# monkey0head/RePlay_cql

Measured on AMD Instinct MI355X. Metric: CQL train-steps/sec, higher is better.
Workload: dtype bf16; 1 GPU; BASELINE.json configs[2]: synthetic 1000000 users x 100000 items, CQL d=128, L=50, B=4096/GPU, bf16 MFMA + fp32 accumulate; users=1000000, items=100000, d=128, window=50, batch_per_gpu=4096, global_batch=4096, parallelism=dp1 (users sharded by rank, RCCL gradient all-reduce), k=10, dp_variant=single

## Files before the change

### include/cqlrec.h

```cpp
#ifndef CQLREC_H
#define CQLREC_H
#include <stdint.h>
#ifdef __cplusplus
extern "C" {
#endif

#define CQLREC_OK 0
#define CQLREC_ERR_INVALID (-1)
#define CQLREC_ERR_HIP (-2)
#define CQLREC_ABI_VERSION 2
#define CQLREC_SEG_ALIGN 64

typedef void* cqlrec_stream;

int cqlrec_abi_version(void);
const char* cqlrec_last_error(void);

typedef struct cqlrec_layout {
  int64_t n_items;
  int32_t d;
  int32_t reserved;
  int64_t off_E_in, off_E_out, off_b_out, off_W1, off_b1, off_W2, off_b2;
  int64_t total;
} cqlrec_layout;
// ... 65 lines not shown
                           cqlrec_stream stream);

int cqlrec_adam_ema(float* theta, float* grads, float* m, float* v, float* target, uint16_t* theta_b,
                    uint16_t* target_b, int64_t n, float step_size, float sqrt_bc2, float beta1, float beta2,
                    float eps, float tau, int32_t zero_grads, cqlrec_stream stream);
int cqlrec_cast_bf16(const float* src, uint16_t* dst_b, int64_t n, cqlrec_stream stream);

int64_t cqlrec_topk_ws_bytes(int64_t n_users, int64_t n_cand, int32_t d, int32_t k);
int cqlrec_score_topk(const uint16_t* H_b, int64_t n_users, const uint16_t* E_b, const float* b, int64_t n_cand,
                      int32_t d, const int32_t* item_ids, const int64_t* seen_off, const int32_t* seen_items,
                      const int32_t* seen_rows, int32_t k, void* ws, int64_t ws_bytes, int32_t* out_idx,
                      float* out_val, int32_t* out_cnt, cqlrec_stream stream);
#define CQLREC_TOPK_ALL 0
#define CQLREC_TOPK_SEEN 1
#define CQLREC_TOPK_SCORE 2
#define CQLREC_TOPK_SEEN_BESIDE 3
int cqlrec_score_topk_phase(const uint16_t* H_b, int64_t n_users, const uint16_t* E_b, const float* b, int64_t n_cand,
                            int32_t d, const int32_t* item_ids, const int64_t* seen_off, const int32_t* seen_items,
                            const int32_t* seen_rows, int32_t k, void* ws, int64_t ws_bytes, int32_t* out_idx,
                            float* out_val, int32_t* out_cnt, int32_t phase, cqlrec_stream stream);

int cqlrec_topk_seen_form(const void* ws, int64_t n_users, int64_t n_cand, int32_t d, int32_t k,
                          int32_t* out , cqlrec_stream stream);

#define CQLREC_SIM_DOT 0
#define CQLREC_SIM_COSINE 1
#define CQLREC_SIM_EUCLID 2
#define CQLREC_ITEM_KNN_MAX_K 512
int cqlrec_item_norms(const uint16_t* E_b, int64_t n_rows, int32_t d, float* norms, cqlrec_stream stream);
int64_t cqlrec_item_knn_ws_bytes(int64_t n_query, int64_t n_cand, int32_t d, int32_t k);
int cqlrec_item_knn(const uint16_t* E_b, const float* norms, int64_t n_rows, int32_t d, const int32_t* query_rows,
                    int64_t n_query, const int32_t* cand_rows, int64_t n_cand, int32_t metric, int32_t k, void* ws,
                    int64_t ws_bytes, int32_t* out_idx, float* out_val, int32_t* out_cnt, cqlrec_stream stream);

#define CQLREC_PAIRS_MAX_K 512
int64_t cqlrec_pairs_topk_ws_bytes(int64_t n_sel, int64_t nnz, int32_t d, int32_t k);
int cqlrec_pairs_topk(const uint16_t* H_b, const uint16_t* E_b, const float* b, int64_t n_items, int32_t d,
                      const int64_t* pair_off, const int32_t* pair_items, const int32_t* rows, int64_t n_sel,
                      const int64_t* seen_off, const int32_t* seen_items, int32_t k, void* ws, int64_t ws_bytes,
                      float* out_score, int32_t* out_idx, float* out_val, int32_t* out_cnt, cqlrec_stream stream);

typedef struct cqlrec_train_ctx {
  cqlrec_layout layout;
  const int64_t* offsets;
  const int32_t* items;
  const float* rewards;
// ... 350 lines not shown
```

### replay_cql_amd/build.py

```python
from __future__ import annotations

import os
import shutil
import subprocess
import sys
from concurrent.futures import ThreadPoolExecutor
from pathlib import Path

PKG = Path(__file__).resolve().parent
CSRC = PKG / "csrc"
LIB = PKG / "libcqlrec.so"
TORCH_LIB = PKG / "libcqlrec_torch.so"
SOURCES = ["library.hip", "state_side.hip", "adam.hip", "qhead.hip", "qhead_de.hip", "qhead_de2.hip", "qhead_de3.hip", "qhead_argmax2.hip", "qhead_fwd2.hip", "qhead_fwd3.hip", "qhead_topk2.hip", "qhead_topk4.hip", "select_common.hip", "segment_common.hip", "topk.hip", "item_knn.hip", "pairs_topk.hip", "gbwd.hip", "prep.hip", "metrics.hip", "split.hip", "prepare.hip", "features.hip", "neighbour.hip", "als.hip", "dense.hip", "slim.hip", "step_streams.hip", "train.hip"]
EXTRA = {
    "state_side.hip": ["-ffp-contract=off"],
    "adam.hip": ["-ffp-contract=off"],
    "qhead.hip": ["-mllvm", "-amdgpu-mfma-vgpr-form=1"],
    "qhead_de.hip": ["-mllvm", "-amdgpu-mfma-vgpr-form=1"],
    "qhead_de2.hip": ["-mllvm", "-amdgpu-mfma-vgpr-form=1"],
    "qhead_de3.hip": ["-mllvm", "-amdgpu-mfma-vgpr-form=1"],
    "qhead_argmax2.hip": ["-mllvm", "-amdgpu-mfma-vgpr-form=1"],
    "qhead_topk2.hip": ["-mllvm", "-amdgpu-mfma-vgpr-form=1"],
    "qhead_topk4.hip": ["-mllvm", "-amdgpu-mfma-vgpr-form=1"],
    "qhead_fwd2.hip": ["-mllvm", "-amdgpu-mfma-vgpr-form=1"],
    "qhead_fwd3.hip": ["-mllvm", "-amdgpu-mfma-vgpr-form=1"],
    "topk.hip": ["-mllvm", "-amdgpu-mfma-vgpr-form=1"],
    "item_knn.hip": ["-ffp-contract=off", "-mllvm", "-amdgpu-mfma-vgpr-form=1"],
    "pairs_topk.hip": ["-ffp-contract=off"],
    "split.hip": ["-ffp-contract=off"],
    "prepare.hip": ["-ffp-contract=off"],
    "features.hip": ["-ffp-contract=off"],
    "neighbour.hip": ["-ffp-contract=off"],
    "als.hip": ["-ffp-contract=off"],
    "dense.hip": ["-ffp-contract=off", "-mllvm", "-amdgpu-mfma-vgpr-form=1"],
    "slim.hip": ["-ffp-contract=off"],
}
ARCH = "gfx950"


def _hipcc() -> str:
    for cand in (os.environ.get("HIPCC"), shutil.which("hipcc"), "/opt/rocm/bin/hipcc"):
        if cand and Path(cand).exists():
            return cand
    raise RuntimeError("hipcc not found (set HIPCC or install ROCm)")


# ... 99 lines not shown
```

### replay_cql_amd/csrc/qhead_internal.h

```cpp
#pragma once
#include "common.h"
#include "qde_pieces.h"

#define QM_LSE 1
#define QM_ARGMAX 2
#define QM_TILEMAX 3
#define QM_BWD_DH 4
#define QM_LSE_DH 6
#define QM_TOPK 7
#define QM_TOPK10 8
#define QS_TOPK_K 16
#define QS_TOPK_BUF 4

#define QS_TI 64
#define QS_SPW_FWD 2
#define QS_SPW_BWD 1
#define QS_TARGET_BLOCKS 768
#define QS_TARGET_BLOCKS_BWD 512
#define QS_REF_MARGIN 5.5f
#ifndef QS_NBUF
#define QS_NBUF 3
#endif
#ifndef QS_NBUF_BWD
#define QS_NBUF_BWD 2
// ... 47 lines not shown
                   int accumulate, hipStream_t s, CqlAdamFix* defer = nullptr, const float* nlse_nat = nullptr);

int cql_qde_fixup_deferred(const CqlAdamFix& f, float* out, float* out_cs, hipStream_t s);
int cql_qhead_bwd_items_long(const uint16_t* H_b, const float* nlse2, const float* coef, const int32_t* act, int64_t batch,
                             const uint16_t* E_out_b, const float* b_out, int64_t n_items, int32_t d, float scale, void* ws,
                             int64_t ws_bytes, float* g_E_out, float* g_b_out, hipStream_t stream, CqlAdamFix* defer,
                             const float* nlse_nat);

struct QTk2Args {
  const uint16_t* H_b;
  int64_t n_users;
  const uint16_t* E_b;
  const float* bias;
  int64_t n_cand;
  int64_t split_rows;
  int nsplit;
  const uint32_t* seen_bits;
  unsigned long long* keys;
  int k;
  const uint32_t* seen_lists;
  const uint16_t* seen_lists_ovf;
  const uint32_t* guard;
  int guard_want;
};
bool cql_topk2_supported(int d, int k, int64_t n_cand);
void cql_topk2_split(int64_t n_users, int64_t n_cand, int* nsplit, int64_t* split_rows);
int64_t cql_topk2_bits_bytes(int64_t n_users, int64_t n_cand);
const uint32_t* cql_topk2_lists_word(const uint32_t* bits, int64_t n_users, int64_t n_cand);
int cql_topk2_seen_bits(const int64_t* seen_off, const int32_t* seen_items, const int32_t* seen_rows, int64_t n_users,
                        int64_t n_cand, uint32_t* bits, hipStream_t s, int beside_scoring = 0);
int cql_topk2_run(const QTk2Args& a, int d, hipStream_t s);
bool cql_topk4_use(int d, int k, int64_t n_users, int64_t n_cand);
int cql_topk4_run(const QTk2Args& a, hipStream_t s);
bool cql_topk4_lists_on();
bool cql_topk4_lists_fit(int64_t n_users, int64_t n_cand, int64_t space_bytes);
int cql_topk4_seen_lists(const int64_t* seen_off, const int32_t* seen_items, const int32_t* seen_rows, int64_t n_users,
                         int64_t n_cand, void* space, int64_t space_bytes, uint32_t* flag, hipStream_t s);

int cql_qhead_argmax_step(const uint16_t* H_b, int64_t rows, const uint16_t* E_out_b, const float* b_out, int64_t n_items,
                          int32_t d, void* ws, int64_t ws_bytes, float* out_val, int32_t* out_idx, hipStream_t stream);

struct QFwd2Args {
  const uint16_t* H_b;
  int64_t n_states;
  const uint16_t* E_b;
  const float* bias;
  int64_t n_items;
// ... 16 lines not shown
```

### replay_cql_amd/csrc/qhead_topk2.hip

```cpp
#include <stdlib.h>
#include <type_traits>
#include "qhead_image.h"

#define TK2_Q 24
#define TK2_K 16
#define TK2_NBUF 3
static_assert(TK2_K == QS_TOPK_K, "list format shared with topk_merge_kernel");

typedef __attribute__((address_space(3))) unsigned long long lds_u64;
typedef __attribute__((ext_vector_type(2))) unsigned int u32x2;
typedef __attribute__((address_space(3))) u32x2 lds_u2;

template <int D>
struct Tk2Cfg {
  using C = DeCfg<D, 4>;
  static constexpr int STRIPS = 4 * 256;
  static constexpr int SEEN = 4 * 512;
  static constexpr int BUF = C::STAGE_BYTES + STRIPS + SEEN;
  static constexpr int RING = TK2_NBUF * BUF;
  static constexpr int QUEUES = 4 * 2 * TK2_Q * 512;
  static constexpr int SMEM = RING + QUEUES;
  static constexpr int VPS = C::LPS + 2;
};

// ... 32 lines not shown
template <int D, int KC>
__global__ __launch_bounds__(256, 1) void qtopk2_kernel(QTk2Args a) {
  static_assert(KC == 10 || KC == 16, "lists of 10 or 16 sorted keys");
  using T = Tk2Cfg<D>;
  using C = typename T::C;
  constexpr int KS = C::KS;
  static_assert(C::TILES == 2 && T::VPS == 6, "two tiles per stage, six pieces per wave (tk2_wait_stages)");
  extern __shared__ __attribute__((aligned(16))) unsigned char smem[];

  const int tid = threadIdx.x, lane = tid & 63;
  const int wave = __builtin_amdgcn_readfirstlane(tid >> 6);
  const int r = lane & 31, h = lane >> 5;
  const int split = blockIdx.x % a.nsplit;
  const int64_t rblk = blockIdx.x / a.nsplit;
  const int64_t res0 = rblk * 256 + wave * 64;
  const int64_t s_begin = (int64_t)split * a.split_rows;
  const int64_t s_end = (s_begin + a.split_rows < a.n_cand) ? (s_begin + a.split_rows) : a.n_cand;
  const int nstage = (s_end > s_begin) ? (int)((s_end - s_begin + C::TI - 1) / C::TI) : 0;
  const uint32_t gstage0 = (uint32_t)(s_begin / C::TI);

  bf16x8 rf[2][KS];
#pragma unroll
  for (int g = 0; g < 2; ++g) load_owner_frags<D>(a.H_b, res0 + g * 32 + r, a.n_users, h, rf[g]);
  owner_fence();

  __amdgpu_buffer_rsrc_t rs_e = make_rsrc(a.E_b, a.n_cand * C::ROWB), rs_b = make_rsrc(a.bias, a.n_cand * 4);
  const int64_t nst_all = (a.n_cand + C::TI - 1) / C::TI;
  const bool has_seen = a.seen_bits != nullptr && res0 < a.n_users;
  const uint32_t* wsrc = has_seen ? a.seen_bits + (res0 >> 6) * nst_all * 128 : (const uint32_t*)a.bias;
  __amdgpu_buffer_rsrc_t rs_w =
      make_rsrc(wsrc, has_seen ? nst_all * 512 : 0);
  const uint32_t voff = img_stage_voff<C>(lane, wave, 0);
  const uint32_t voff4 = (uint32_t)lane * 4;
  const uint32_t smem_base = lds_addr_of(smem);
  auto issue_piece = [&](int stage, int buf, int pc) __attribute__((always_inline)) {
    const uint32_t bufp = __builtin_amdgcn_readfirstlane(smem_base + buf * T::BUF);
    const uint32_t gs = gstage0 + (uint32_t)stage;
    if (pc < C::LPS) bdma16(voff, rs_e, gs * C::STAGE_BYTES + C::PSTEP * pc, bufp + (4 * pc + wave) * 1024);
    else if (pc == C::LPS) bdma4(voff4, rs_b, gs * (C::TI * 4), bufp + C::STAGE_BYTES + wave * 256);
    else bdma16_lo32(4 * voff4, rs_w, gs * 512, bufp + C::STAGE_BYTES + T::STRIPS + wave * 512);
  };
  auto issue = [&](int stage, int buf) __attribute__((always_inline)) {
#pragma unroll
    for (int pc = 0; pc < T::VPS; ++pc) issue_piece(stage, buf, pc);
  };

// ... 1 lines not shown
  const ImgRead o = img_read_offsets<C>(lane);
  const int oa0 = o.oa0, oa1 = o.oa1;
  const int os = C::STAGE_BYTES + wave * 256 + 16 * h;
  const int ow = C::STAGE_BYTES + T::STRIPS + wave * 512 + r * 8;
  const lds_u8 *pA0, *pA1, *pS, *pW;
  const lds_u8 *nA0, *nA1, *nS;
  int boff_c = 0, boff_n = T::BUF;
  auto set_ptrs = [&]() __attribute__((always_inline)) {
    pA0 = lbase + boff_c + oa0; pA1 = lbase + boff_c + oa1; pS = lbase + boff_c + os; pW = lbase + boff_c + ow;
    nA0 = lbase + boff_n + oa0; nA1 = lbase + boff_n + oa1; nS = lbase + boff_n + os;
  };
  set_ptrs();

  lds_u8* qb[2];
  uint32_t la[2][2 * TK2_K];
  float thr[2];
  int cnt[2];
#pragma unroll
  for (int g = 0; g < 2; ++g) {
    qb[g] = (lds_u8*)smem + T::RING + ((wave * 2 + g) * TK2_Q * 64 + lane) * 8;
#ifdef TK2_ABL_NOSLOW
    thr[g] = 3.0e38f;
#else
    thr[g] = -3.0e38f;
#endif
    cnt[g] = 0;
#pragma unroll
    for (int j = 0; j < 2 * TK2_K; ++j) TK2_AW(la[g][j], 0u);
  }
  const int kth = a.k - 1;
  const bool kb0 = kth & 1, kb1 = kth & 2, kb2 = kth & 4, kb3 = kth & 8;

  auto merge = [&](auto G_) __attribute__((always_inline)) {
    constexpr int g = decltype(G_)::value;
    unsigned long long lst[TK2_K];
#pragma unroll
    for (int j = 0; j < TK2_K; ++j) {
      if (j < KC) {
        uint32_t lo, hi;
        TK2_AR(lo, la[g][2 * j]);
        TK2_AR(hi, la[g][2 * j + 1]);
        lst[j] = ((unsigned long long)hi << 32) | lo;
      } else {
        lst[j] = 0ull;
      }
    }
#pragma unroll 1
// ... 6 lines not shown
        kx = gt ? lst[j] : kx;
        lst[j] = hi_;
      }
    }
#pragma unroll
    for (int j = 0; j < KC; ++j) {
      TK2_AW(la[g][2 * j], (uint32_t)lst[j]);
      TK2_AW(la[g][2 * j + 1], (uint32_t)(lst[j] >> 32));
    }
    cnt[g] = 0;
    const unsigned long long m0 = kb0 ? ~0ull : 0ull, m1 = kb1 ? ~0ull : 0ull, m2 = kb2 ? ~0ull : 0ull,
                             m3 = kb3 ? ~0ull : 0ull;
    unsigned long long t8[8], t4[4], t2[2];
#pragma unroll
    for (int j = 0; j < 8; ++j) t8[j] = (lst[2 * j + 1] & m0) | (lst[2 * j] & ~m0);
#pragma unroll
    for (int j = 0; j < 4; ++j) t4[j] = (t8[2 * j + 1] & m1) | (t8[2 * j] & ~m1);
#pragma unroll
    for (int j = 0; j < 2; ++j) t2[j] = (t4[2 * j + 1] & m2) | (t4[2 * j] & ~m2);
    const unsigned long long kk = (t2[1] & m3) | (t2[0] & ~m3);
    const uint32_t okey = (uint32_t)(kk >> 32);
    const float own = (kk != 0ull) ? f32_from_order_key(okey) : -3.0e38f;
    const float own_up = (kk != 0ull) ? f32_from_order_key(okey + 1u) : -3.0e38f;
    thr[g] = fmaxf(own_up, __shfl_xor(own, 32));
  };

  auto slow = [&](const f32x16& acc, auto G_, int64_t trow0, uint32_t w) __attribute__((always_inline)) {
    constexpr int g = decltype(G_)::value;
    if (__builtin_amdgcn_ballot_w64(cnt[g] > TK2_Q - 16) != 0) merge(G_);
    float qm[4];
#pragma unroll
    for (int q = 0; q < 4; ++q) qm[q] = tk2_max4(acc[4 * q], acc[4 * q + 1], acc[4 * q + 2], acc[4 * q + 3]);
    const uint32_t wh = w >> (4 * h);
    const int lim = (int)((s_end - trow0 < 64) ? (s_end - trow0) : 64) - 4 * h;
    const uint32_t nrow = ~((uint32_t)trow0 + 4u * (uint32_t)h);
#pragma unroll
    for (int q = 0; q < 4; ++q) {
      if (__builtin_amdgcn_ballot_w64(qm[q] >= thr[g]) == 0) continue;
#pragma unroll
      for (int jj = 0; jj < 4; ++jj) {
        const int i = 4 * q + jj;
        const int rc = 8 * q + jj;
        const bool c0 = acc[i] >= thr[g];
        if (__builtin_amdgcn_ballot_w64(c0) == 0) continue;
        if (c0) {
          uint32_t whv = wh, nrv = nrow;
          int limv = lim;
// ... 298 lines not shown
```

### replay_cql_amd/csrc/qhead_topk4.hip

```cpp
#include <stdlib.h>
#include <type_traits>
#include "qhead_image.h"

#define TK4_G 4
#define TK4_Q 12
#define TK4_K 16
#define TK4_NBUF 3
#define TK4_SLOT_WORDS 64
#define TK4_SLOT_CAP 124
static_assert(TK4_K == QS_TOPK_K, "list format shared with topk_merge_kernel");

typedef __attribute__((address_space(3))) unsigned long long lds_u64_4;
typedef __attribute__((ext_vector_type(2))) unsigned int u32x2_4;
typedef __attribute__((address_space(3))) u32x2_4 lds_u2_4;
typedef __attribute__((address_space(3))) unsigned int lds_u32_4;
typedef __attribute__((address_space(3))) u32x4 lds_u4_4;

template <int D>
struct Tk4Cfg {
  using C = DeCfg<D, 4>;
  static constexpr int STRIP = 256;
  static constexpr int SEEN = 4 * 1024;
  static constexpr int BUF = C::STAGE_BYTES + STRIP + SEEN;
  static constexpr int RING = TK4_NBUF * BUF;
// ... 33 lines not shown
  using C = typename T::C;
  constexpr int KS = C::KS;
  static_assert(D == 128 && C::TILES == 2 && C::LPS == 4, "d = 128: two tiles per stage, four row pieces per wave");
  extern __shared__ __attribute__((aligned(16))) unsigned char smem[];

  const int tid = threadIdx.x, lane = tid & 63;
  const int wave = __builtin_amdgcn_readfirstlane(tid >> 6);
  const int r = lane & 31, h = lane >> 5;
  const int split = blockIdx.x % a.nsplit;
  const int64_t rblk = blockIdx.x / a.nsplit;
  const int64_t res0 = rblk * 512 + wave * 128;
  const int64_t s_begin = (int64_t)split * a.split_rows;
  const int64_t s_end = (s_begin + a.split_rows < a.n_cand) ? (s_begin + a.split_rows) : a.n_cand;
  const int nstage = (s_end > s_begin) ? (int)((s_end - s_begin + C::TI - 1) / C::TI) : 0;
  const uint32_t gstage0 = (uint32_t)(s_begin / C::TI);

  u32x4 rfa[TK4_G][KS];
#pragma unroll
  for (int g = 0; g < TK4_G; ++g) {
    int64_t row = res0 + g * 32 + r;
    if (row >= a.n_users) row = a.n_users - 1;
#pragma unroll
    for (int s = 0; s < KS; ++s) rfa[g][s] = *reinterpret_cast<const u32x4*>(a.H_b + row * D + 16 * s + 8 * h);
  }
  owner_fence();

  __amdgpu_buffer_rsrc_t rs_e = make_rsrc(a.E_b, a.n_cand * C::ROWB), rs_b = make_rsrc(a.bias, a.n_cand * 4);
  const int64_t nst_all = (a.n_cand + C::TI - 1) / C::TI;
  const int64_t nblk64 = LISTS ? (a.n_users + 127) / 128 : (a.n_users + 63) / 64;
  const int64_t blk0 = LISTS ? (res0 >> 7) : (res0 >> 6);
  const uint32_t* const seen_src = LISTS ? a.seen_lists : a.seen_bits;
  const bool has_seen = seen_src != nullptr && blk0 < nblk64;
  const uint32_t* wsrc = has_seen ? seen_src + blk0 * nst_all * (LISTS ? 64 : 128) : (const uint32_t*)a.bias;
  const bool two_blocks = !LISTS && has_seen && (blk0 + 1 < nblk64);
  const int64_t w_records = has_seen ? (LISTS ? nst_all * 256 : (two_blocks ? 2 : 1) * nst_all * 512) : 0;
  const uint64_t wp = (uint64_t)wsrc;
  const uint64_t wp_u = ((uint64_t)(uint32_t)__builtin_amdgcn_readfirstlane((int)(uint32_t)(wp >> 32)) << 32) |
                        (uint32_t)__builtin_amdgcn_readfirstlane((int)(uint32_t)wp);
  __amdgpu_buffer_rsrc_t rs_w = __builtin_amdgcn_make_buffer_rsrc((void*)wp_u, 0, __builtin_amdgcn_readfirstlane((int)w_records),
                                                                  0x00020000);
  const uint32_t voff_w = LISTS ? (uint32_t)lane * 4u
                                : (uint32_t)((lane >> 5) * (uint32_t)(nst_all * 512) + (lane & 31) * 16);
  const uint32_t voff = img_stage_voff<C>(lane, wave, 0);
  const uint32_t voff4 = (uint32_t)lane * 4;
  const uint32_t smem_base = lds_addr_of(smem);
  auto issue_piece = [&](int stage, int buf, int pc) __attribute__((always_inline)) {
// ... 11 lines not shown
  const lds_u8* lbase = (const lds_u8*)smem;
  const ImgRead o = img_read_offsets<C>(lane);
  const int oa0 = o.oa0, oa1 = o.oa1;
  const int os = C::STAGE_BYTES + 16 * h;
  const int ow = C::STAGE_BYTES + T::STRIP + wave * 1024 + r * 8;
  const lds_u8 *pA0, *pA1, *pS, *pW;
  const lds_u8 *nA0, *nA1, *nS;
  int boff_c = 0, boff_n = T::BUF;
  auto set_ptrs = [&]() __attribute__((always_inline)) {
    pA0 = lbase + boff_c + oa0; pA1 = lbase + boff_c + oa1; pS = lbase + boff_c + os; pW = lbase + boff_c + ow;
    nA0 = lbase + boff_n + oa0; nA1 = lbase + boff_n + oa1; nS = lbase + boff_n + os;
  };
  set_ptrs();

  uint32_t la[TK4_G][2 * TK4_K];
  float thr[TK4_G];
  int cnt[TK4_G];
  lds_u8* const qb0 = (lds_u8*)smem + T::RING + ((wave * TK4_G) * TK4_Q * 64 + lane) * 8;
#pragma unroll
  for (int g = 0; g < TK4_G; ++g) {
#ifdef TK4_ABL_NOSLOW
    thr[g] = 3.0e38f;
#else
    thr[g] = -3.0e38f;
#endif
    cnt[g] = 0;
#pragma unroll
    for (int j = 0; j < 2 * TK4_K; ++j) TK4_AW(la[g][j], 0u);
  }
  const int kth = a.k - 1;
  const bool kb0 = kth & 1, kb1 = kth & 2, kb2 = kth & 4, kb3 = kth & 8;

  auto merge = [&](auto G_) __attribute__((always_inline)) {
    constexpr int g = decltype(G_)::value;
    lds_u8* const qb = qb0 + g * (TK4_Q * 512);
    unsigned long long lst[TK4_K];
#pragma unroll
    for (int j = 0; j < TK4_K; ++j) {
      if (j < KC) {
        uint32_t lo, hi;
        TK4_AR(lo, la[g][2 * j]);
        TK4_AR(hi, la[g][2 * j + 1]);
        lst[j] = ((unsigned long long)hi << 32) | lo;
      } else {
        lst[j] = 0ull;
      }
    }
// ... 12 lines not shown
    for (int j = 0; j < KC; ++j) {
      TK4_AW(la[g][2 * j], (uint32_t)lst[j]);
      TK4_AW(la[g][2 * j + 1], (uint32_t)(lst[j] >> 32));
    }
    cnt[g] = 0;
    unsigned long long kk;
    if (kth == KC - 1) {
      kk = lst[KC - 1];
    } else {
      const unsigned long long m0 = kb0 ? ~0ull : 0ull, m1 = kb1 ? ~0ull : 0ull, m2 = kb2 ? ~0ull : 0ull,
                               m3 = kb3 ? ~0ull : 0ull;
      unsigned long long t8[8], t4[4], t2[2];
#pragma unroll
      for (int j = 0; j < 8; ++j) t8[j] = (lst[2 * j + 1] & m0) | (lst[2 * j] & ~m0);
#pragma unroll
      for (int j = 0; j < 4; ++j) t4[j] = (t8[2 * j + 1] & m1) | (t8[2 * j] & ~m1);
#pragma unroll
      for (int j = 0; j < 2; ++j) t2[j] = (t4[2 * j + 1] & m2) | (t4[2 * j] & ~m2);
      kk = (t2[1] & m3) | (t2[0] & ~m3);
    }
    const uint32_t okey = (uint32_t)(kk >> 32);
    const float own = (kk != 0ull) ? f32_from_order_key(okey) : -3.0e38f;
    const float own_up = (kk != 0ull) ? f32_from_order_key(okey + 1u) : -3.0e38f;
    thr[g] = fmaxf(own_up, __shfl_xor(own, 32));
  };

  auto slow = [&](const f32x16& acc, auto G_, int64_t trow0, uint32_t w) __attribute__((always_inline)) {
    constexpr int g = decltype(G_)::value;
    lds_u8* const qb = qb0 + g * (TK4_Q * 512);
    const uint32_t wh = w >> (4 * h);
    const int lim = (int)((s_end - trow0 < 64) ? (s_end - trow0) : 64) - 4 * h;
    const uint32_t nrow = ~((uint32_t)trow0 + 4u * (uint32_t)h);
    uint32_t qmask = 0u;
    {
      const float m0 = tk4_max4(acc[0], acc[1], acc[2], acc[3]), m1 = tk4_max4(acc[4], acc[5], acc[6], acc[7]);
      const float m2 = tk4_max4(acc[8], acc[9], acc[10], acc[11]), m3 = tk4_max4(acc[12], acc[13], acc[14], acc[15]);
      qmask = (__builtin_amdgcn_ballot_w64(m0 >= thr[g]) != 0 ? 1u : 0u) | (__builtin_amdgcn_ballot_w64(m1 >= thr[g]) != 0 ? 2u : 0u) |
              (__builtin_amdgcn_ballot_w64(m2 >= thr[g]) != 0 ? 4u : 0u) | (__builtin_amdgcn_ballot_w64(m3 >= thr[g]) != 0 ? 8u : 0u);
    }
#pragma unroll 1
    while (qmask != 0u) {
      const int q = __builtin_ctz(qmask);
      qmask &= qmask - 1u;
      float e[4];
#ifdef TK4_ABL_QUAD_SELECT
      const bool q1 = q & 1, q2 = q & 2;
#pragma unroll
// ... 410 lines not shown
```

### replay_cql_amd/csrc/topk.hip

```cpp
#include <stdlib.h>
#include "qhead_internal.h"
#include "select_common.h"

#define TK_CB_SMALL 1024
#define TK_CB_LARGE 4096
#define TK_MAX_K 2048
#define TK_SEEN_LDS 512

template <int D, int KPL, int TK_CB>
__global__ __launch_bounds__(64) void topk_select_kernel(const uint16_t* __restrict__ H_b, int64_t n_users,
                                                         const uint16_t* __restrict__ E_b, const float* __restrict__ b,
                                                         int64_t n_cand, const int32_t* __restrict__ item_ids,
                                                         const int64_t* __restrict__ seen_off,
                                                         const int32_t* __restrict__ seen_items,
                                                         const int32_t* __restrict__ seen_rows,
                                                         const float* __restrict__ tm_t, int gstride, int ngroups,
                                                         int tg, int k, int32_t* __restrict__ out_idx,
                                                         float* __restrict__ out_val, int32_t* __restrict__ out_cnt) {
  constexpr int KS = D / 16;
  __shared__ uint32_t hist[256];
  __shared__ float scores[32];
  __shared__ uint64_t cand[TK_CB];
  __shared__ int32_t seen_lds[TK_SEEN_LDS];

// ... 449 lines not shown
                            int32_t* out_idx, float* out_val, int32_t* out_cnt, hipStream_t s) {
  if (2 * nsplit <= 4)
    hipLaunchKernelGGL(topk_merge_wave_kernel, dim3(cql_ceil_div(n_users, 4)), dim3(256), 0, s, keys, nsplit, n_users,
                       item_ids, k, out_idx, out_val, out_cnt);
  else
    hipLaunchKernelGGL(topk_merge_kernel, dim3(cql_ceil_div(n_users, 256)), dim3(256), 0, s, keys, nsplit, n_users, item_ids,
                       k, out_idx, out_val, out_cnt);
}

static inline int64_t tk_bits_words(int64_t n_cand) { return ((n_cand + 31) / 32 + 3) / 4 * 4; }
#define TK_FUSED_MAX_SPLIT 32
static QSplit tk_fused_split(int64_t n_cand, int64_t n_users, int d) {
  (void)d;
  QSplit sp = qs_choose_split(n_cand, n_users, 2, QS_TI, 512);
  if (sp.nsplit > TK_FUSED_MAX_SPLIT) {
    const int64_t units = (n_cand + QS_TI - 1) / QS_TI;
    const int64_t upb = (units + TK_FUSED_MAX_SPLIT - 1) / TK_FUSED_MAX_SPLIT;
    sp.split_rows = upb * QS_TI;
    sp.nsplit = (int)((n_cand + sp.split_rows - 1) / sp.split_rows);
  }
  return sp;
}

extern "C" int64_t cqlrec_topk_ws_bytes(int64_t n_users, int64_t n_cand, int32_t d, int32_t k) {
  (void)d;
  (void)k;
  const SelGroups sg = sel_groups(n_cand);
  const int64_t two_pass =
      cql_align256((int64_t)sg.ngroups * n_users * 4) + cql_align256((int64_t)sg.gstride * n_users * 4);
  int64_t fused = cql_align256((int64_t)tk_fused_split(n_cand, n_users, d).nsplit * n_users * 2 * QS_TOPK_K * 8) +
                  cql_align256(n_users * tk_bits_words(n_cand) * 4);
  if (cql_topk2_supported(d, k, n_cand)) {
    int ns;
    int64_t sr;
    cql_topk2_split(n_users, n_cand, &ns, &sr);
    const int64_t f2 =
        cql_align256((int64_t)ns * n_users * 2 * QS_TOPK_K * 8) + cql_align256(cql_topk2_bits_bytes(n_users, n_cand));
    if (f2 > fused) fused = f2;
  }
  return (two_pass > fused ? two_pass : fused) + 256;
}

extern "C" int cqlrec_score_topk(const uint16_t* H_b, int64_t n_users, const uint16_t* E_b, const float* b,
                                 int64_t n_cand, int32_t d, const int32_t* item_ids, const int64_t* seen_off,
                                 const int32_t* seen_items, const int32_t* seen_rows, int32_t k, void* ws,
                                 int64_t ws_bytes, int32_t* out_idx, float* out_val, int32_t* out_cnt,
                                 cqlrec_stream stream) {
  return cqlrec_score_topk_phase(H_b, n_users, E_b, b, n_cand, d, item_ids, seen_off, seen_items, seen_rows, k, ws, ws_bytes,
                                 out_idx, out_val, out_cnt, CQLREC_TOPK_ALL, stream);
}

static bool tk_uses_topk2(int32_t d, int32_t k, int64_t n_cand, const int32_t* item_ids) {
  return item_ids == nullptr && cql_topk2_supported(d, k, n_cand);
}

extern "C" int cqlrec_topk_seen_form(const void* ws, int64_t n_users, int64_t n_cand, int32_t d, int32_t k, int32_t* out,
                                     cqlrec_stream stream) {
  CQL_REQUIRE(ws && out && n_users > 0 && n_cand > 0, "topk_seen_form: bad arguments");
  *out = -1;
  if (!tk_uses_topk2(d, k, n_cand, nullptr)) return CQLREC_OK;
  int ns;
  int64_t sr;
  cql_topk2_split(n_users, n_cand, &ns, &sr);
  const uint32_t* bits = (const uint32_t*)((const char*)ws + cql_align256((int64_t)ns * n_users * 2 * QS_TOPK_K * 8));
  const uint32_t* word = cql_topk2_lists_word(bits, n_users, n_cand);
  if (!word) return CQLREC_OK;
  uint32_t v = 0;
  if (hipMemcpyAsync(&v, word, 4, hipMemcpyDeviceToHost, (hipStream_t)stream) != hipSuccess ||
      hipStreamSynchronize((hipStream_t)stream) != hipSuccess) {
    cql_set_error("topk_seen_form: copying the word back failed");
    return CQLREC_ERR_HIP;
  }
  *out = v ? 1 : 0;
  return CQLREC_OK;
}

extern "C" int cqlrec_score_topk_phase(const uint16_t* H_b, int64_t n_users, const uint16_t* E_b, const float* b,
                                       int64_t n_cand, int32_t d, const int32_t* item_ids, const int64_t* seen_off,
                                       const int32_t* seen_items, const int32_t* seen_rows, int32_t k, void* ws,
                                       int64_t ws_bytes, int32_t* out_idx, float* out_val, int32_t* out_cnt,
                                       int32_t phase, cqlrec_stream stream) {
  CQL_REQUIRE(phase == CQLREC_TOPK_ALL || phase == CQLREC_TOPK_SEEN || phase == CQLREC_TOPK_SCORE ||
                  phase == CQLREC_TOPK_SEEN_BESIDE, "score_topk: phase=%d", phase);
  if (phase == CQLREC_TOPK_SEEN || phase == CQLREC_TOPK_SEEN_BESIDE) {
    CQL_REQUIRE(ws && n_users > 0 && n_cand > 0, "score_topk (seen phase): bad arguments");
    CQL_REQUIRE(ws_bytes >= cqlrec_topk_ws_bytes(n_users, n_cand, d, k), "score_topk: workspace too small");
    if (!seen_off || !tk_uses_topk2(d, k, n_cand, item_ids)) return CQLREC_OK;
    CQL_REQUIRE(seen_items != nullptr, "score_topk: seen_items is NULL");
    int ns;
    int64_t sr;
    cql_topk2_split(n_users, n_cand, &ns, &sr);
    uint32_t* bits = (uint32_t*)((char*)ws + cql_align256((int64_t)ns * n_users * 2 * QS_TOPK_K * 8));
    CqlProfScope prof(CQLREC_PH_TOPK_SELECT, (hipStream_t)stream);
    return cql_topk2_seen_bits(seen_off, seen_items, seen_rows, n_users, n_cand, bits, (hipStream_t)stream,
                               phase == CQLREC_TOPK_SEEN_BESIDE);
  }
// ... 4 lines not shown
  CQL_REQUIRE(seen_off == nullptr || seen_items != nullptr, "score_topk: seen_items is NULL");
  CQL_REQUIRE(ws_bytes >= cqlrec_topk_ws_bytes(n_users, n_cand, d, k), "score_topk: workspace too small");
  hipStream_t s = (hipStream_t)stream;
  if (tk_uses_topk2(d, k, n_cand, item_ids)) {
    QTk2Args a2 = {};
    a2.H_b = H_b;
    a2.n_users = n_users;
    a2.E_b = E_b;
    a2.bias = b;
    a2.n_cand = n_cand;
    a2.k = k;
    cql_topk2_split(n_users, n_cand, &a2.nsplit, &a2.split_rows);
    a2.keys = (unsigned long long*)ws;
    if (seen_off) {
      uint32_t* bits = (uint32_t*)((char*)ws + cql_align256((int64_t)a2.nsplit * n_users * 2 * QS_TOPK_K * 8));
      if (phase == CQLREC_TOPK_ALL) {
        CqlProfScope prof(CQLREC_PH_TOPK_SELECT, s);
        const int rc = cql_topk2_seen_bits(seen_off, seen_items, seen_rows, n_users, n_cand, bits, s);
        if (rc != CQLREC_OK) return rc;
      }
      a2.seen_bits = bits;
      a2.guard = cql_topk2_lists_word(bits, n_users, n_cand);
      a2.seen_lists = a2.guard ? bits : nullptr;
    }
    {
      CqlProfScope prof(CQLREC_PH_TOPK_TILEMAX, s);
      const int rc = cql_topk2_run(a2, d, s);
      if (rc != CQLREC_OK) return rc;
    }
    CqlProfScope prof(CQLREC_PH_TOPK_SELECT, s);
    tk_launch_merge((const unsigned long long*)ws, a2.nsplit, n_users, item_ids, (int)k, out_idx, out_val, out_cnt, s);
    CQL_LAUNCH_CHECK("score_topk (topk2)");
    return CQLREC_OK;
  }
  if (k <= QS_TOPK_K && item_ids == nullptr && n_cand < (1ll << 31)) {
    const QSplit sp = tk_fused_split(n_cand, n_users, d);
    uint32_t* bits = nullptr;
    const int64_t W = tk_bits_words(n_cand);
    if (seen_off) {
      bits = (uint32_t*)((char*)ws + cql_align256((int64_t)sp.nsplit * n_users * 2 * QS_TOPK_K * 8));
      CqlProfScope prof(CQLREC_PH_TOPK_SELECT, s);
      if (hipMemsetAsync(bits, 0, (size_t)n_users * W * 4, s) != hipSuccess) {
        cql_set_error("score_topk: hipMemsetAsync failed");
        return CQLREC_ERR_HIP;
      }
      hipLaunchKernelGGL(topk_seen_bits_kernel, dim3(cql_ceil_div(n_users, 4)), dim3(256), 0, s, seen_off, seen_items,
// ... 60 lines not shown
```

Measured before the change: 1540 train-steps/s (B=4096 transitions per step and GPU).

## Seed top-k threshold per user with a pilot pass over likely candidates

Adds a pilot stage ahead of the fused scoring top-k. It scores all items against the mean user vector, picks roughly 256 promising items by radix select, then computes each user's exact k-th best unseen score over that subset with MFMA. The topk2/topk4 kernels use this as the starting threshold and as a floor, so fewer candidates take the slow insertion path. It costs three extra kernel launches, extra workspace, and a per-threshold-update global load with a vmcnt wait. The affected code is the top-k scoring path, which may not be part of the CQL train step.

```diff
diff --git a/include/cqlrec.h b/include/cqlrec.h
--- a/include/cqlrec.h
+++ b/include/cqlrec.h
@@ -111,6 +111,10 @@
 
 int cqlrec_topk_seen_form(const void* ws, int64_t n_users, int64_t n_cand, int32_t d, int32_t k,
                           int32_t* out , cqlrec_stream stream);
+
+int cqlrec_topk_pilot_set(int32_t mode);
+int cqlrec_topk_pilot_tau(const void* ws, int64_t n_users, int64_t n_cand, int32_t d, int32_t k,
+                          float* out , cqlrec_stream stream);
 
 #define CQLREC_SIM_DOT 0
 #define CQLREC_SIM_COSINE 1
diff --git a/replay_cql_amd/build.py b/replay_cql_amd/build.py
--- a/replay_cql_amd/build.py
+++ b/replay_cql_amd/build.py
@@ -11,7 +11,7 @@
 CSRC = PKG / "csrc"
 LIB = PKG / "libcqlrec.so"
 TORCH_LIB = PKG / "libcqlrec_torch.so"
-SOURCES = ["library.hip", "state_side.hip", "adam.hip", "qhead.hip", "qhead_de.hip", "qhead_de2.hip", "qhead_de3.hip", "qhead_argmax2.hip", "qhead_fwd2.hip", "qhead_fwd3.hip", "qhead_topk2.hip", "qhead_topk4.hip", "select_common.hip", "segment_common.hip", "topk.hip", "item_knn.hip", "pairs_topk.hip", "gbwd.hip", "prep.hip", "metrics.hip", "split.hip", "prepare.hip", "features.hip", "neighbour.hip", "als.hip", "dense.hip", "slim.hip", "step_streams.hip", "train.hip"]
+SOURCES = ["library.hip", "state_side.hip", "adam.hip", "qhead.hip", "qhead_de.hip", "qhead_de2.hip", "qhead_de3.hip", "qhead_argmax2.hip", "qhead_fwd2.hip", "qhead_fwd3.hip", "qhead_topk2.hip", "qhead_topk4.hip", "qhead_topk_pilot.hip", "select_common.hip", "segment_common.hip", "topk.hip", "item_knn.hip", "pairs_topk.hip", "gbwd.hip", "prep.hip", "metrics.hip", "split.hip", "prepare.hip", "features.hip", "neighbour.hip", "als.hip", "dense.hip", "slim.hip", "step_streams.hip", "train.hip"]
 EXTRA = {
     "state_side.hip": ["-ffp-contract=off"],
     "adam.hip": ["-ffp-contract=off"],
@@ -22,6 +22,7 @@
     "qhead_argmax2.hip": ["-mllvm", "-amdgpu-mfma-vgpr-form=1"],
     "qhead_topk2.hip": ["-mllvm", "-amdgpu-mfma-vgpr-form=1"],
     "qhead_topk4.hip": ["-mllvm", "-amdgpu-mfma-vgpr-form=1"],
+    "qhead_topk_pilot.hip": ["-mllvm", "-amdgpu-mfma-vgpr-form=1"],
     "qhead_fwd2.hip": ["-mllvm", "-amdgpu-mfma-vgpr-form=1"],
     "qhead_fwd3.hip": ["-mllvm", "-amdgpu-mfma-vgpr-form=1"],
     "topk.hip": ["-mllvm", "-amdgpu-mfma-vgpr-form=1"],
diff --git a/replay_cql_amd/csrc/qhead_internal.h b/replay_cql_amd/csrc/qhead_internal.h
--- a/replay_cql_amd/csrc/qhead_internal.h
+++ b/replay_cql_amd/csrc/qhead_internal.h
@@ -93,7 +93,14 @@
   const uint16_t* seen_lists_ovf;
   const uint32_t* guard;
   int guard_want;
+  const float* tau0;
 };
+#define CQL_TOPK_PILOT_MAX 512
+bool cql_topk_pilot_on();
+int64_t cql_topk_pilot_bytes(int64_t n_users, int64_t n_cand);
+int cql_topk_pilot_run(const QTk2Args& a, const int64_t* seen_off, const int32_t* seen_items, const int32_t* seen_rows,
+                       void* region, hipStream_t s, const float** tau0);
+const float* cql_topk_pilot_tau(const void* region);
 bool cql_topk2_supported(int d, int k, int64_t n_cand);
 void cql_topk2_split(int64_t n_users, int64_t n_cand, int* nsplit, int64_t* split_rows);
 int64_t cql_topk2_bits_bytes(int64_t n_users, int64_t n_cand);
diff --git a/replay_cql_amd/csrc/qhead_topk2.hip b/replay_cql_amd/csrc/qhead_topk2.hip
--- a/replay_cql_amd/csrc/qhead_topk2.hip
+++ b/replay_cql_amd/csrc/qhead_topk2.hip
@@ -78,6 +78,13 @@
   bf16x8 rf[2][KS];
 #pragma unroll
   for (int g = 0; g < 2; ++g) load_owner_frags<D>(a.H_b, res0 + g * 32 + r, a.n_users, h, rf[g]);
+  float tau_g[2];
+#pragma unroll
+  for (int g = 0; g < 2; ++g) {
+    int64_t row = res0 + g * 32 + r;
+    if (row >= a.n_users) row = a.n_users - 1;
+    tau_g[g] = a.tau0 != nullptr ? a.tau0[row] : -3.0e38f;
+  }
   owner_fence();
 
   __amdgpu_buffer_rsrc_t rs_e = make_rsrc(a.E_b, a.n_cand * C::ROWB), rs_b = make_rsrc(a.bias, a.n_cand * 4);
@@ -125,7 +132,7 @@
 #ifdef TK2_ABL_NOSLOW
     thr[g] = 3.0e38f;
 #else
-    thr[g] = -3.0e38f;
+    thr[g] = tau_g[g];
 #endif
     cnt[g] = 0;
 #pragma unroll
@@ -178,7 +185,16 @@
     const uint32_t okey = (uint32_t)(kk >> 32);
     const float own = (kk != 0ull) ? f32_from_order_key(okey) : -3.0e38f;
     const float own_up = (kk != 0ull) ? f32_from_order_key(okey + 1u) : -3.0e38f;
-    thr[g] = fmaxf(own_up, __shfl_xor(own, 32));
+    float floor_ = -3.0e38f;
+    if (a.tau0 != nullptr) {
+      int rr = r;
+      asm volatile("" : "+v"(rr));
+      int64_t row = res0 + g * 32 + rr;
+      if (row >= a.n_users) row = a.n_users - 1;
+      floor_ = a.tau0[row];
+      asm volatile("s_waitcnt vmcnt(0)" ::: "memory");
+    }
+    thr[g] = fmaxf(fmaxf(own_up, __shfl_xor(own, 32)), floor_);
   };
 
   auto slow = [&](const f32x16& acc, auto G_, int64_t trow0, uint32_t w) __attribute__((always_inline)) {
diff --git a/replay_cql_amd/csrc/qhead_topk4.hip b/replay_cql_amd/csrc/qhead_topk4.hip
--- a/replay_cql_amd/csrc/qhead_topk4.hip
+++ b/replay_cql_amd/csrc/qhead_topk4.hip
@@ -79,6 +79,13 @@
     if (row >= a.n_users) row = a.n_users - 1;
 #pragma unroll
     for (int s = 0; s < KS; ++s) rfa[g][s] = *reinterpret_cast<const u32x4*>(a.H_b + row * D + 16 * s + 8 * h);
+  }
+  float tau_g[TK4_G];
+#pragma unroll
+  for (int g = 0; g < TK4_G; ++g) {
+    int64_t row = res0 + g * 32 + r;
+    if (row >= a.n_users) row = a.n_users - 1;
+    tau_g[g] = a.tau0 != nullptr ? a.tau0[row] : -3.0e38f;
   }
   owner_fence();
 
@@ -136,7 +143,7 @@
 #ifdef TK4_ABL_NOSLOW
     thr[g] = 3.0e38f;
 #else
-    thr[g] = -3.0e38f;
+    thr[g] = tau_g[g];
 #endif
     cnt[g] = 0;
 #pragma unroll
@@ -195,7 +202,16 @@
     const uint32_t okey = (uint32_t)(kk >> 32);
     const float own = (kk != 0ull) ? f32_from_order_key(okey) : -3.0e38f;
     const float own_up = (kk != 0ull) ? f32_from_order_key(okey + 1u) : -3.0e38f;
-    thr[g] = fmaxf(own_up, __shfl_xor(own, 32));
+    float floor_ = -3.0e38f;
+    if (a.tau0 != nullptr) {
+      int rr = r;
+      asm volatile("" : "+v"(rr));
+      int64_t row = res0 + g * 32 + rr;
+      if (row >= a.n_users) row = a.n_users - 1;
+      floor_ = a.tau0[row];
+      asm volatile("s_waitcnt vmcnt(0)" ::: "memory");
+    }
+    thr[g] = fmaxf(fmaxf(own_up, __shfl_xor(own, 32)), floor_);
   };
 
   auto slow = [&](const f32x16& acc, auto G_, int64_t trow0, uint32_t w) __attribute__((always_inline)) {
diff --git a/replay_cql_amd/csrc/qhead_topk_pilot.hip b/replay_cql_amd/csrc/qhead_topk_pilot.hip
--- /dev/null
+++ b/replay_cql_amd/csrc/qhead_topk_pilot.hip
@@ -0,0 +1,388 @@
+#include <stdlib.h>
+#include "qhead_image.h"
+
+#define TKP_SAMPLE 128
+#define TKP_ROWB 272
+#define TKP_WAVES 8
+#define TKP_NONE 0xFFFFu
+
+typedef __attribute__((address_space(3))) unsigned int lds_u32_p;
+typedef __attribute__((address_space(3))) u32x4 lds_u4_p;
+
+__global__ __launch_bounds__(256) void tkp_score_kernel(const uint16_t* __restrict__ H_b, int64_t n_users,
+                                                        const uint16_t* __restrict__ E_b, const float* __restrict__ b,
+                                                        int64_t n_cand, float* __restrict__ score) {
+  __shared__ float part[4][128];
+  __shared__ float mean[128];
+  const int t = threadIdx.x, c2 = t & 63, rg = t >> 6;
+  const int64_t S = n_users < TKP_SAMPLE ? n_users : TKP_SAMPLE, stride = n_users / S;
+  float s0 = 0.f, s1 = 0.f;
+  for (int64_t i = rg; i < S; i += 4) {
+    const uint32_t w = reinterpret_cast<const uint32_t*>(H_b)[i * stride * 64 + c2];
+    s0 += __uint_as_float(w << 16);
+    s1 += __uint_as_float(w & 0xFFFF0000u);
+  }
+  part[rg][2 * c2] = s0;
+  part[rg][2 * c2 + 1] = s1;
+  __syncthreads();
+  if (t < 128) mean[t] = (part[0][t] + part[1][t] + part[2][t] + part[3][t]) / (float)S;
+  __syncthreads();
+  const int64_t c = (int64_t)blockIdx.x * 256 + t;
+  if (c >= n_cand) return;
+  const uint4* row = reinterpret_cast<const uint4*>(E_b + c * 128);
+  float acc = b[c];
+#pragma unroll
+  for (int ch = 0; ch < 16; ++ch) {
+    float e[8];
+    unpack_bf16x8(row[ch], e);
+#pragma unroll
+    for (int j = 0; j < 8; ++j) acc = fmaf(e[j], mean[8 * ch + j], acc);
+  }
+  score[c] = acc;
+}
+
+__device__ __forceinline__ void tkp_pick_bin(const uint32_t* hist, uint32_t need, uint32_t* s_bin, uint32_t* s_need) {
+  const int lane = threadIdx.x;
+  uint32_t c[4], tot = 0u;
+#pragma unroll
+  for (int j = 0; j < 4; ++j) {
+    c[j] = hist[255 - 4 * lane - j];
+    tot += c[j];
+  }
+  uint32_t incl = tot;
+#pragma unroll
+  for (int o = 1; o < 64; o <<= 1) {
+    const uint32_t v = __shfl_up(incl, o);
+    if (lane >= o) incl += v;
+  }
+  uint32_t cum = incl - tot;
+  if (cum < need && need <= incl) {
+#pragma unroll
+    for (int j = 0; j < 4; ++j) {
+      if (cum < need && need <= cum + c[j]) {
+        *s_bin = (uint32_t)(255 - 4 * lane - j);
+        *s_need = need - cum;
+      }
+      cum += c[j];
+    }
+  }
+}
+
+__global__ __launch_bounds__(1024) void tkp_select_kernel(const float* __restrict__ score, int64_t n_cand, int P,
+                                                          int32_t* __restrict__ pid, uint16_t* __restrict__ pos,
+                                                          int32_t* __restrict__ np_out) {
+  __shared__ uint32_t hist[256];
+  __shared__ uint32_t s_bin, s_need;
+  __shared__ uint32_t wcnt[16];
+  const int t = threadIdx.x, lane = t & 63, wave = t >> 6;
+  const bool all = n_cand <= P;
+  uint32_t t16 = 0u;
+  if (!all) {
+    const int64_t stride = n_cand >= 64ll * P ? 8 : 1;
+    const int64_t m = (n_cand + stride - 1) / stride;
+    uint32_t need = stride == 1 ? (uint32_t)P : (uint32_t)(3 * P / 32 > 0 ? 3 * P / 32 : 1);
+    uint32_t prefix = 0u;
+    for (int pass = 0; pass < 2; ++pass) {
+      const int shift = pass ? 16 : 24;
+      if (t < 256) hist[t] = 0u;
+      if (t == 0) { s_bin = 0u; s_need = 0u; }
+      __syncthreads();
+      for (int64_t i = t; i < m; i += 1024) {
+        const uint32_t key = f32_order_key(score[i * stride]);
+        if (pass == 0 || (key >> 24) == prefix) atomicAdd(&hist[(key >> shift) & 255u], 1u);
+      }
+      __syncthreads();
+      if (t < 64) tkp_pick_bin(hist, need, &s_bin, &s_need);
+      __syncthreads();
+      prefix = (prefix << 8) | s_bin;
+      need = s_need;
+      __syncthreads();
+    }
+    t16 = prefix;
+  }
+  const int64_t per = ((n_cand + 15) / 16 + 63) / 64 * 64;
+  const int64_t w_lo = (int64_t)wave * per < n_cand ? (int64_t)wave * per : n_cand;
+  const int64_t w_hi = w_lo + per < n_cand ? w_lo + per : n_cand;
+  auto taken = [&](int64_t i) -> bool { return i < w_hi && (all || (f32_order_key(score[i]) >> 16) >= t16); };
+  uint32_t c = 0u;
+  for (int64_t i0 = w_lo; i0 < w_hi; i0 += 64) c += (uint32_t)__builtin_popcountll(__builtin_amdgcn_ballot_w64(taken(i0 + lane)));
+  if (lane == 0) wcnt[wave] = c;
+  __syncthreads();
+  uint32_t base = 0u, total = 0u;
+  for (int w = 0; w < 16; ++w) {
+    if (w < wave) base += wcnt[w];
+    total += wcnt[w];
+  }
+  for (int64_t i0 = w_lo; i0 < w_hi; i0 += 64) {
+    const int64_t i = i0 + lane;
+    const bool tk = taken(i);
+    const unsigned long long mk = __builtin_amdgcn_ballot_w64(tk);
+    const uint32_t rank = base + (uint32_t)__builtin_popcountll(mk & ((1ull << lane) - 1ull));
+    if (i < w_hi) {
+      const bool in = tk && rank < (uint32_t)P;
+      if (in) pid[rank] = (int32_t)i;
+      pos[i] = in ? (uint16_t)rank : (uint16_t)TKP_NONE;
+    }
+    base += (uint32_t)__builtin_popcountll(mk);
+  }
+  if (t == 0) *np_out = (int32_t)(total < (uint32_t)P ? total : (uint32_t)P);
+}
+
+struct TkPilotArgs {
+  const uint16_t* H_b;
+  int64_t n_users;
+  const uint16_t* E_b;
+  const float* bias;
+  int64_t n_cand;
+  const int64_t* seen_off;
+  const int32_t* seen_items;
+  const int32_t* seen_rows;
+  const int32_t* pid;
+  const uint16_t* pos;
+  const int32_t* np;
+  int np_max;
+  int k;
+  float* tau0;
+};
+
+#define TKP_CE(a, b)                            \
+  do {                                          \
+    const uint32_t hi__ = (a) > (b) ? (a) : (b); \
+    const uint32_t lo__ = (a) > (b) ? (b) : (a); \
+    (a) = hi__;                                 \
+    (b) = lo__;                                 \
+  } while (0)
+__device__ __forceinline__ void tkp_bitonic_merge16(uint32_t (&v)[16]) {
+#pragma unroll
+  for (int j = 8; j > 0; j >>= 1)
+#pragma unroll
+    for (int i = 0; i < 16; ++i)
+      if ((i ^ j) > i) TKP_CE(v[i], v[i ^ j]);
+}
+__device__ __forceinline__ void tkp_sort16(uint32_t (&v)[16]) {
+#pragma unroll
+  for (int k = 2; k <= 16; k <<= 1)
+#pragma unroll
+    for (int j = k >> 1; j > 0; j >>= 1)
+#pragma unroll
+      for (int i = 0; i < 16; ++i) {
+        const int l = i ^ j;
+        if (l > i) {
+          if ((i & k) == 0) TKP_CE(v[i], v[l]);
+          else TKP_CE(v[l], v[i]);
+        }
+      }
+}
+
+__global__ __launch_bounds__(TKP_WAVES * 64, 4) void tkp_tau_kernel(TkPilotArgs a) {
+  extern __shared__ __attribute__((aligned(16))) unsigned char smem[];
+  const int tid = threadIdx.x, lane = tid & 63;
+  const int wave = __builtin_amdgcn_readfirstlane(tid >> 6);
+  const int r = lane & 31, h = lane >> 5;
+  int np = __builtin_amdgcn_readfirstlane(*a.np);
+  np = np < 1 ? 1 : np > a.np_max ? a.np_max : np;
+  const int nt = (np + 31) / 32, rows = nt * 32;
+  lds_u8* const lrows = (lds_u8*)smem;
+  lds_u8* const lbias = lrows + rows * TKP_ROWB;
+  lds_u8* const mW = lbias + rows * 4 + wave * (rows * 4);
+
+  for (int i = tid; i < rows * 16; i += TKP_WAVES * 64) {
+    const int row = i >> 4, ch = i & 15;
+    const int64_t item = a.pid[row < np ? row : np - 1];
+    *(lds_u4_p*)(lrows + row * TKP_ROWB + 16 * ch) = *reinterpret_cast<const u32x4*>(a.E_b + item * 128 + 8 * ch);
+  }
+  for (int i = tid; i < rows; i += TKP_WAVES * 64)
+    *(__attribute__((address_space(3))) float*)(lbias + 4 * i) = a.bias[a.pid[i < np ? i : np - 1]];
+  __syncthreads();
+
+  const int64_t ngroups = (a.n_users + 31) / 32;
+  const int kth = a.k - 1;
+  for (int64_t grp = (int64_t)blockIdx.x * TKP_WAVES + wave; grp < ngroups; grp += (int64_t)gridDim.x * TKP_WAVES) {
+    const int64_t urow = grp * 32 + r;
+    bf16x8 rf[8];
+    load_owner_frags<128>(a.H_b, urow, a.n_users, h, rf);
+
+    for (int i = lane; i < rows; i += 64) *(lds_u32_p*)(mW + 4 * i) = 0u;
+    if (a.seen_off != nullptr) {
+      int64_t lo = 0;
+      uint32_t len = 0u;
+      if (urow < a.n_users) {
+        const int64_t srow = a.seen_rows ? (int64_t)a.seen_rows[urow] : urow;
+        lo = a.seen_off[srow];
+        const int64_t n = a.seen_off[srow + 1] - lo;
+        len = n > 0 ? (uint32_t)n : 0u;
+      }
+      uint32_t incl = len;
+#pragma unroll
+      for (int o = 1; o < 32; o <<= 1) {
+        const uint32_t v = __shfl_up(incl, o, 32);
+        if (r >= o) incl += v;
+      }
+      const uint32_t pre = incl - len;
+      const uint32_t total = __shfl(incl, 31);
+      for (uint32_t base = 0u; base < total; base += 256u) {
+        int32_t id[4];
+        int usr[4];
+#pragma unroll
+        for (int q = 0; q < 4; ++q) {
+          const uint32_t f = base + 64u * q + (uint32_t)lane;
+          int p = 0;
+#pragma unroll
+          for (int step = 16; step >= 1; step >>= 1) {
+            const uint32_t probe = __shfl(pre, p + step);
+            if (probe <= f) p += step;
+          }
+          const int64_t lo_u = __shfl(lo, p);
+          const uint32_t pre_u = __shfl(pre, p);
+          usr[q] = p;
+          id[q] = f < total ? a.seen_items[lo_u + (int64_t)(f - pre_u)] : -1;
+        }
+        uint32_t where[4];
+#pragma unroll
+        for (int q = 0; q < 4; ++q)
+          where[q] = (id[q] >= 0 && (int64_t)id[q] < a.n_cand) ? (uint32_t)a.pos[id[q]] : TKP_NONE;
+#pragma unroll
+        for (int q = 0; q < 4; ++q)
+          if (where[q] < (uint32_t)np)
+            __hip_atomic_fetch_or((lds_u32_p*)(mW + 4 * ((where[q] >> 5) * 32 + usr[q])), 1u << (where[q] & 31u),
+                                  __ATOMIC_RELAXED, __HIP_MEMORY_SCOPE_WAVEFRONT);
+      }
+    }
+    __builtin_amdgcn_fence(__ATOMIC_ACQ_REL, "wavefront");
+
+    uint32_t best[16];
+#pragma unroll
+    for (int j = 0; j < 16; ++j) best[j] = 0u;
+    for (int t = 0; t < nt; ++t) {
+      f32x16 acc;
+#pragma unroll
+      for (int q = 0; q < 4; ++q) {
+        const f32x4 b4 = *(const lds_f4*)(lbias + 4 * (32 * t + 8 * q + 4 * h));
+        acc[4 * q + 0] = b4[0];
+        acc[4 * q + 1] = b4[1];
+        acc[4 * q + 2] = b4[2];
+        acc[4 * q + 3] = b4[3];
+      }
+      const lds_u8* const arow = lrows + (32 * t + r) * TKP_ROWB + 16 * h;
+#pragma unroll
+      for (int s = 0; s < 8; ++s)
+        acc = __builtin_amdgcn_mfma_f32_32x32x16_bf16(*(const lds_bf16x8*)(arow + 32 * s), rf[s], acc, 0, 0, 0);
+      const uint32_t wh = *(const lds_u32_p*)(mW + 4 * (32 * t + r)) >> (4 * h);
+      const int lim = np - 32 * t - 4 * h;
+      uint32_t key[16];
+#pragma unroll
+      for (int i = 0; i < 16; ++i) {
+        const int rc = 8 * (i >> 2) + (i & 3);
+        key[i] = (((wh >> rc) & 1u) == 0u && rc < lim) ? f32_order_key(acc[i]) : 0u;
+      }
+      tkp_sort16(key);
+#pragma unroll
+      for (int j = 0; j < 16; ++j) best[j] = best[j] > key[15 - j] ? best[j] : key[15 - j];
+      tkp_bitonic_merge16(best);
+    }
+    uint32_t other[16];
+#pragma unroll
+    for (int j = 0; j < 16; ++j) other[j] = __shfl_xor(best[j], 32);
+#pragma unroll
+    for (int j = 0; j < 16; ++j) best[j] = best[j] > other[15 - j] ? best[j] : other[15 - j];
+    tkp_bitonic_merge16(best);
+    uint32_t kk = 0u;
+#pragma unroll
+    for (int j = 0; j < 16; ++j) kk = (j == kth) ? best[j] : kk;
+    const float v = f32_from_order_key(kk);
+    if (h == 0 && urow < a.n_users) a.tau0[urow] = (kk != 0u && v > -3.0e38f) ? v : -3.0e38f;
+    __builtin_amdgcn_fence(__ATOMIC_ACQ_REL, "wavefront");
+  }
+}
+
+static int g_pilot_mode = -1;
+
+extern "C" int cqlrec_topk_pilot_set(int32_t mode) {
+  CQL_REQUIRE(mode == 0 || mode == 1, "topk_pilot_set: mode=%d (0 or 1)", mode);
+  g_pilot_mode = mode;
+  return CQLREC_OK;
+}
+
+bool cql_topk_pilot_on() {
+  if (g_pilot_mode < 0) {
+    const char* v = getenv("CQL_TOPK_PILOT");
+    g_pilot_mode = (v && *v == '0') ? 0 : 1;
+  }
+  return g_pilot_mode != 0;
+}
+
+static int tkp_size() {
+  static const int p = [] {
+    int v = getenv("CQL_TOPK_PILOT_P") ? atoi(getenv("CQL_TOPK_PILOT_P")) : 256;
+    v = v / 32 * 32;
+    return v < 32 ? 32 : v > CQL_TOPK_PILOT_MAX ? CQL_TOPK_PILOT_MAX : v;
+  }();
+  return p;
+}
+
+struct TkPilotWs {
+  float* tau0;
+  int32_t* pid;
+  uint16_t* pos;
+  float* score;
+};
+static TkPilotWs tkp_carve(void* region, int64_t n_users, int64_t n_cand) {
+  TkPilotWs w;
+  char* p = (char*)region;
+  w.tau0 = (float*)p;     p += cql_align256(n_users * 4);
+  w.pid = (int32_t*)p;    p += cql_align256(CQL_TOPK_PILOT_MAX * 4 + 4);
+  w.pos = (uint16_t*)p;   p += cql_align256(n_cand * 2);
+  w.score = (float*)p;
+  return w;
+}
+int64_t cql_topk_pilot_bytes(int64_t n_users, int64_t n_cand) {
+  return cql_align256(n_users * 4) + cql_align256(CQL_TOPK_PILOT_MAX * 4 + 4) + cql_align256(n_cand * 2) + cql_align256(n_cand * 4);
+}
+const float* cql_topk_pilot_tau(const void* region) { return (const float*)region; }
+
+int cql_topk_pilot_run(const QTk2Args& a, const int64_t* seen_off, const int32_t* seen_items, const int32_t* seen_rows,
+                       void* region, hipStream_t s, const float** tau0) {
+  const TkPilotWs w = tkp_carve(region, a.n_users, a.n_cand);
+  const int P = tkp_size();
+  const int np = a.n_cand < P ? (int)a.n_cand : P;
+  if (a.n_cand > P)
+    hipLaunchKernelGGL(tkp_score_kernel, dim3((unsigned)((a.n_cand + 255) / 256)), dim3(256), 0, s, a.H_b, a.n_users, a.E_b,
+                       a.bias, a.n_cand, w.score);
+  hipLaunchKernelGGL(tkp_select_kernel, dim3(1), dim3(1024), 0, s, (const float*)w.score, a.n_cand, P, w.pid, w.pos,
+                     w.pid + CQL_TOPK_PILOT_MAX);
+  TkPilotArgs t = {};
+  t.H_b = a.H_b;
+  t.n_users = a.n_users;
+  t.E_b = a.E_b;
+  t.bias = a.bias;
+  t.n_cand = a.n_cand;
+  t.seen_off = seen_off;
+  t.seen_items = seen_items;
+  t.seen_rows = seen_rows;
+  t.pid = w.pid;
+  t.pos = w.pos;
+  t.np = w.pid + CQL_TOPK_PILOT_MAX;
+  t.np_max = np;
+  t.k = a.k;
+  t.tau0 = w.tau0;
+  const int rows = (np + 31) / 32 * 32;
+  const int smem = rows * TKP_ROWB + rows * 4 + TKP_WAVES * rows * 4;
+  static bool attr_set_dev[CQL_MAX_DEVICES] = {};
+  static int cus_dev[CQL_MAX_DEVICES] = {};
+  const int slot = cql_device_slot();
+  if (!attr_set_dev[slot]) {
+    (void)hipFuncSetAttribute((const void*)tkp_tau_kernel, hipFuncAttributeMaxDynamicSharedMemorySize,
+                              CQL_TOPK_PILOT_MAX * (TKP_ROWB + 4 + TKP_WAVES * 4));
+    int dev = 0;
+    (void)hipGetDevice(&dev);
+    if (hipDeviceGetAttribute(&cus_dev[slot], hipDeviceAttributeMultiprocessorCount, dev) != hipSuccess || cus_dev[slot] <= 0)
+      cus_dev[slot] = 256;
+    attr_set_dev[slot] = true;
+  }
+  const int64_t want = ((a.n_users + 31) / 32 + TKP_WAVES - 1) / TKP_WAVES;
+  const int64_t cap = (int64_t)cus_dev[slot] * (2 * smem <= 160 * 1024 ? 2 : 1);
+  hipLaunchKernelGGL(tkp_tau_kernel, dim3((unsigned)(want < cap ? want : cap)), dim3(TKP_WAVES * 64), smem, s, t);
+  CQL_LAUNCH_CHECK("topk pilot");
+  *tau0 = w.tau0;
+  return CQLREC_OK;
+}
diff --git a/replay_cql_amd/csrc/topk.hip b/replay_cql_amd/csrc/topk.hip
--- a/replay_cql_amd/csrc/topk.hip
+++ b/replay_cql_amd/csrc/topk.hip
@@ -495,9 +495,7 @@
   return sp;
 }
 
-extern "C" int64_t cqlrec_topk_ws_bytes(int64_t n_users, int64_t n_cand, int32_t d, int32_t k) {
-  (void)d;
-  (void)k;
+static int64_t tk_ws_forms_bytes(int64_t n_users, int64_t n_cand, int32_t d, int32_t k) {
   const SelGroups sg = sel_groups(n_cand);
   const int64_t two_pass =
       cql_align256((int64_t)sg.ngroups * n_users * 4) + cql_align256((int64_t)sg.gstride * n_users * 4);
@@ -512,6 +510,11 @@
     if (f2 > fused) fused = f2;
   }
   return (two_pass > fused ? two_pass : fused) + 256;
+}
+
+extern "C" int64_t cqlrec_topk_ws_bytes(int64_t n_users, int64_t n_cand, int32_t d, int32_t k) {
+  return tk_ws_forms_bytes(n_users, n_cand, d, k) +
+         (cql_topk2_supported(d, k, n_cand) ? cql_topk_pilot_bytes(n_users, n_cand) : 0);
 }
 
 extern "C" int cqlrec_score_topk(const uint16_t* H_b, int64_t n_users, const uint16_t* E_b, const float* b,
@@ -545,6 +548,19 @@
     return CQLREC_ERR_HIP;
   }
   *out = v ? 1 : 0;
+  return CQLREC_OK;
+}
+
+extern "C" int cqlrec_topk_pilot_tau(const void* ws, int64_t n_users, int64_t n_cand, int32_t d, int32_t k, float* out,
+                                     cqlrec_stream stream) {
+  CQL_REQUIRE(ws && out && n_users > 0 && n_cand > 0, "topk_pilot_tau: bad arguments");
+  CQL_REQUIRE(tk_uses_topk2(d, k, n_cand, nullptr), "topk_pilot_tau: d=%d k=%d: this shape runs no pilot", d, k);
+  const float* tau0 = cql_topk_pilot_tau((const char*)ws + tk_ws_forms_bytes(n_users, n_cand, d, k));
+  if (hipMemcpyAsync(out, tau0, (size_t)n_users * 4, hipMemcpyDeviceToHost, (hipStream_t)stream) != hipSuccess ||
+      hipStreamSynchronize((hipStream_t)stream) != hipSuccess) {
+    cql_set_error("topk_pilot_tau: copying tau0 back failed");
+    return CQLREC_ERR_HIP;
+  }
   return CQLREC_OK;
 }
 
@@ -595,6 +611,12 @@
       a2.seen_bits = bits;
       a2.guard = cql_topk2_lists_word(bits, n_users, n_cand);
       a2.seen_lists = a2.guard ? bits : nullptr;
+    }
+    if (cql_topk_pilot_on()) {
+      CqlProfScope prof(CQLREC_PH_TOPK_SELECT, s);
+      const int rc = cql_topk_pilot_run(a2, seen_off, seen_items, seen_rows, (char*)ws + tk_ws_forms_bytes(n_users, n_cand, d, k),
+                                        s, &a2.tau0);
+      if (rc != CQLREC_OK) return rc;
     }
     {
       CqlProfScope prof(CQLREC_PH_TOPK_TILEMAX, s);
```

Result: no change. 1537 train-steps/s (B=4096 transitions per step and GPU), median of 2 (-0.2%).
